# gisbi-kim/lt-mapper

Measured on AMD Instinct MI355X. Metric: keyframe-pairs/sec (removert+diff), higher is better.
Workload: dtype f32; 1 GPU; lot-2x500-os1-64-3res; sensor=os1-64

## Files before the change

### include/ltm.h

```cpp
#ifndef LTM_H
#define LTM_H

#include <stddef.h>
#include <stdint.h>

#ifdef __cplusplus
extern "C" {
#endif

#define LTM_ABI_VERSION 1

enum {
    LTM_OK = 0,
    LTM_E_INVALID = -1,
    LTM_E_DEVICE = -2,
    LTM_E_NOMEM = -3,
    LTM_E_UNSUPPORTED = -4
};

typedef struct ltm_ctx ltm_ctx;
typedef uint64_t ltm_cloud;
typedef uint64_t ltm_scanset;
typedef uint64_t ltm_poses;

// ... 158 lines not shown
int  ltm_icp_align_plane_scanset(ltm_ctx*, size_t n_pairs, ltm_search* const* targets, ltm_scanset sources, const uint32_t* source_kf ,
                                 const double* init16_or_null, const ltm_icp_params*, ltm_icp_result* results_host, double* trace_host_or_null);

int ltm_pose6d_to_affine3f(const float* xyzrpy , size_t n, float* affine12 );
int ltm_submaps_assemble(ltm_ctx*, ltm_scanset scans, const float* affine12_host_or_null ,
                         const int32_t* keys_host, size_t n_windows, int search_num, float leaf, int order, ltm_scanset* out);
int ltm_search_build_scanset(ltm_ctx*, ltm_scanset, size_t kf_begin, size_t kf_end, ltm_search** out );

typedef struct ltm_event ltm_event;
int  ltm_lane_create(ltm_ctx* parent, ltm_ctx** lane);
int  ltm_lane_fence(ltm_ctx* done_in, ltm_ctx* before_next_of);
int  ltm_event_record(ltm_ctx*, ltm_event** ev);
int  ltm_event_wait(ltm_ctx*, ltm_event* ev);
void ltm_event_destroy(ltm_event* ev);
int  ltm_cloud_lend(ltm_ctx* from, ltm_cloud h, ltm_ctx* to, ltm_cloud* out);
int  ltm_cloud_give(ltm_ctx* from, ltm_cloud h, ltm_ctx* to, ltm_cloud* out);
int  ltm_scanset_lend(ltm_ctx* from, ltm_scanset h, ltm_ctx* to, ltm_scanset* out);
int  ltm_scanset_give(ltm_ctx* from, ltm_scanset h, ltm_ctx* to, ltm_scanset* out);
int ltm_debug_range_image(ltm_ctx*, ltm_cloud pts, const double* T1, const double* T2, float res_alpha,
                          float* rimg, int32_t* ptidx);
int ltm_debug_viz_images(ltm_ctx*, ltm_cloud map, ltm_scanset scans, ltm_poses poses, size_t kf, float res_alpha, int mode,
                         float range_min, float range_max, float diff_min, float diff_max,
                         uint8_t* scan_bgr, uint8_t* map_bgr, uint8_t* diff_bgr, uint8_t* ptidx_bgr);
int ltm_debug_project(ltm_ctx*, const float* xyz, size_t n, float res_alpha, float* out_az_el_r, int32_t* out_row_col);
void ltm_rimg_size(float vfov, float hfov, float res_alpha, int* rows, int* cols);
int ltm_debug_selfcheck(ltm_ctx*, uint64_t* mismatches3, int* fast_math_enabled);
int ltm_debug_elevation_fit(float vfov_deg, float* c4, double* max_err_rad);
int ltm_debug_pcl_sort_order(const uint32_t* leaf_idx, size_t n, uint32_t* order_out, int use_std_sort, uint32_t* heap_sort_fallbacks );
int ltm_debug_voxel_key_bits(const float* mn3, const float* mx3, float leaf, uint64_t* kept_mask, unsigned* depth, double* frame_min3);
int ltm_debug_proj_launch(float vfov, float hfov, float res_alpha, const double* base2lidar16_or_null, size_t map_points, size_t n_keyframes, int on_device,
                          float* out_f32, uint32_t* out_u32, uint32_t first_block, size_t n_blocks, uint32_t* out_tile, uint32_t* out_kf);
int ltm_debug_vote_run_launch(size_t map_points, size_t n_keyframes, int tile_run, uint32_t first_block, size_t n_blocks, uint32_t* out_run, uint32_t* out_kf,
                              uint32_t* out_run_len, uint32_t* out_grid);
int ltm_debug_cull_check(ltm_ctx*, const float* xyz, size_t n, const double* inv_pose16_or_null, float res_alpha, uint64_t* violations);
int ltm_debug_cull_validation(ltm_ctx*, uint64_t* shapes_checked, uint64_t* shapes_failed);
int ltm_debug_occlusion_stats(ltm_ctx*, uint64_t* pairs, uint64_t* first_shell, uint64_t* projected, int reset);
int ltm_debug_voxel_stats(ltm_ctx*, uint64_t* grids, uint64_t* identity_hits, int reset);
int ltm_debug_knn_stats(ltm_ctx*, uint64_t* queries, uint64_t* undecided, uint64_t* two_phase_calls, uint64_t* unsorted_queue_calls, int reset);
int ltm_debug_sc_paths(int num_ring, int num_sector, int* scatter_in_lds, int* pair_in_lds);
int ltm_debug_cull_stats(ltm_ctx*, uint64_t* survivors, uint64_t* points, int reset);
int ltm_debug_pool_live(ltm_ctx*, uint64_t* live_blocks, uint64_t* live_bytes);

int ltm_profile_enable(ltm_ctx*, int on);
int ltm_profile_reset(ltm_ctx*);
int ltm_profile_read(ltm_ctx*, const char** names, double* ms, uint64_t* launches, double* units, double* bytes, int cap);
int ltm_profile_read_compulsory(ltm_ctx*, double* bytes_c, int cap);

#ifdef __cplusplus
}
#endif
#endif
```

### lt-mapper_amd/capi.py

```python
import ctypes as C
import os

import numpy as np

_HERE = os.path.dirname(os.path.abspath(__file__))
LIB_PATH = os.path.join(_HERE, "libltm_hip.so")

_lib = None

LTM_OK = 0
ERR_NAMES = {0: "LTM_OK", -1: "LTM_E_INVALID", -2: "LTM_E_DEVICE", -3: "LTM_E_NOMEM", -4: "LTM_E_UNSUPPORTED"}


class LtmError(RuntimeError):
    def __init__(self, code, msg):
        super().__init__(f"{ERR_NAMES.get(code, code)}: {msg}")
        self.code = code


class LtmConfig(C.Structure):
    _fields_ = [("vfov", C.c_float), ("hfov", C.c_float), ("lidar2base", C.c_double * 16),
                ("device", C.c_int), ("max_kf_batch", C.c_int)]


# ... 103 lines not shown
    "ltm_search_result_info": (_i, [_vp, _vp, _psz, _psz, C.POINTER(_vp), C.POINTER(_vp), C.POINTER(_vp)]),
    "ltm_search_result_free": (_i, [_vp, _vp]),
    "ltm_search_estimate_normals": (_i, [_vp, _sz, C.POINTER(_vp), _i, _vp]),
    "ltm_search_normals_info": (_i, [_vp, _vp, C.POINTER(_i), C.POINTER(_vp)]),
    "ltm_search_normals_download": (_i, [_vp, _vp, _vp]),
    "ltm_sc_default_params": (None, [C.POINTER(ScParams)]),
    "ltm_sc_from_scanset": (_i, [_vp, _u64, _sz, _sz, C.POINTER(ScParams), C.POINTER(_vp)]),
    "ltm_sc_from_descriptors": (_i, [_vp, _vp, _sz, C.POINTER(ScParams), C.POINTER(_vp)]),
    "ltm_sc_info": (_i, [_vp, _vp, _psz, C.POINTER(_i), C.POINTER(_i)]),
    "ltm_sc_download": (_i, [_vp, _vp, _vp, _vp, _vp]),
    "ltm_sc_distance": (_i, [_vp, _vp, _vp, _vp, _sz, C.POINTER(ScParams), _vp, _vp]),
    "ltm_sc_detect": (_i, [_vp, _vp, _vp, C.POINTER(ScParams), _vp, _vp, _vp, _vp, _vp]),
    "ltm_sc_free": (_i, [_vp, _vp]),
    "ltm_icp_default_params": (None, [C.POINTER(IcpParams)]),
    "ltm_icp_align": (_i, [_vp, _sz, C.POINTER(_vp), _pu64, _vp, C.POINTER(IcpParams), _vp, _vp]),
    "ltm_icp_align_scanset": (_i, [_vp, _sz, C.POINTER(_vp), _u64, _vp, _vp, C.POINTER(IcpParams), _vp, _vp]),
    "ltm_icp_align_plane": (_i, [_vp, _sz, C.POINTER(_vp), _pu64, _vp, C.POINTER(IcpParams), _vp, _vp]),
    "ltm_icp_align_plane_scanset": (_i, [_vp, _sz, C.POINTER(_vp), _u64, _vp, _vp, C.POINTER(IcpParams), _vp, _vp]),
    "ltm_pose6d_to_affine3f": (_i, [_vp, _sz, _vp]),
    "ltm_submaps_assemble": (_i, [_vp, _u64, _vp, _vp, _sz, _i, _f, _i, _pu64]),
    "ltm_search_build_scanset": (_i, [_vp, _u64, _sz, _sz, C.POINTER(_vp)]),
    "ltm_debug_pool_live": (_i, [_vp, _pu64, _pu64]),
    "ltm_debug_range_image": (_i, [_vp, _u64, _vp, _vp, _f, _vp, _vp]),
    "ltm_debug_viz_images": (_i, [_vp, _u64, _u64, _u64, _sz, _f, _i, _f, _f, _f, _f, _vp, _vp, _vp, _vp]),
    "ltm_debug_project": (_i, [_vp, _vp, _sz, _f, _vp, _vp]),
    "ltm_debug_elevation_fit": (_i, [_f, C.POINTER(_f), C.POINTER(C.c_double)]),
    "ltm_debug_pcl_sort_order": (_i, [C.POINTER(C.c_uint32), C.c_size_t, C.POINTER(C.c_uint32), _i, C.POINTER(C.c_uint32)]),
    "ltm_debug_voxel_key_bits": (_i, [C.POINTER(_f), C.POINTER(_f), _f, _pu64, C.POINTER(C.c_uint), C.POINTER(C.c_double)]),
    "ltm_debug_selfcheck": (_i, [_vp, _pu64, C.POINTER(_i)]),
    "ltm_debug_cull_check": (_i, [_vp, _vp, _sz, _vp, _f, _pu64]),
    "ltm_debug_cull_stats": (_i, [_vp, _pu64, _pu64, _i]),
    "ltm_debug_proj_launch": (_i, [_f, _f, _f, _vp, _sz, _sz, _i, _vp, _vp, C.c_uint32, _sz, _vp, _vp]),
    "ltm_debug_vote_run_launch": (_i, [_sz, _sz, _i, C.c_uint32, _sz, _vp, _vp, _vp, _vp]),
    "ltm_debug_cull_validation": (_i, [_vp, _pu64, _pu64]),
    "ltm_debug_occlusion_stats": (_i, [_vp, _pu64, _pu64, _pu64, _i]),
    "ltm_debug_voxel_stats": (_i, [_vp, _pu64, _pu64, _i]),
    "ltm_debug_knn_stats": (_i, [_vp, _pu64, _pu64, _pu64, _pu64, _i]),
    "ltm_debug_sc_paths": (_i, [_i, _i, C.POINTER(_i), C.POINTER(_i)]),
    "ltm_rimg_size": (None, [_f, _f, _f, C.POINTER(_i), C.POINTER(_i)]),
    "ltm_profile_enable": (_i, [_vp, _i]),
    "ltm_profile_reset": (_i, [_vp]),
    "ltm_profile_read_compulsory": (_i, [_vp, C.POINTER(C.c_double), _i]),
    "ltm_profile_read": (_i, [_vp, C.POINTER(C.c_char_p), C.POINTER(C.c_double), _pu64, C.POINTER(C.c_double),
                              C.POINTER(C.c_double), _i]),
}


def load_library(path=None):
    global _lib
    if _lib is not None and path is None:
        return _lib
    p = path or LIB_PATH
    try:
        import torch
    except Exception:
        pass
    if not os.path.exists(p):
        raise FileNotFoundError(
            f"{p} not found: build it with `make hip` (or __graft_entry__.build()). There is no CPU fallback.")
    lib = C.CDLL(p)
    for name, (res, args) in SIGNATURES.items():
        fn = getattr(lib, name)
        fn.restype = res
        fn.argtypes = args
    if path is None:
        _lib = lib
# ... 7 lines not shown
    if n < 0:
        raise ValueError("unsupported box / leaf")
    return n, mask.value, depth.value, np.array(list(fmin))


PROJ_LAUNCH_F32 = ("half_v", "half_h", "inv_v", "inv_h", "frows", "fcols", "row_max", "col_max", "row_scale", "col_scale", "row_bias", "col_bias",
                   "certain_lim", "rmin2", "eps", "el_tclamp")
PROJ_LAUNCH_U32 = ("rows", "cols", "npx", "steep_clamps", "packable", "n_tiles", "n_tg", "tg_magic", "tg_shift", "grid", "el_fit", "fast")


def proj_launch(vfov, hfov, alpha, base2lidar=None, map_points=0, n_keyframes=1, on_device=False, first_block=0, n_blocks=0):
    f = np.zeros(len(PROJ_LAUNCH_F32), dtype=np.float32)
    u = np.zeros(len(PROJ_LAUNCH_U32), dtype=np.uint32)
    tile = np.zeros(max(n_blocks, 1), dtype=np.uint32)
    kf = np.zeros(max(n_blocks, 1), dtype=np.uint32)
    b2l = None if base2lidar is None else _mat16(base2lidar)
    rc = load_library().ltm_debug_proj_launch(float(vfov), float(hfov), float(alpha), None if b2l is None else b2l.ctypes.data, int(map_points),
                                              int(n_keyframes), int(bool(on_device)), f.ctypes.data, u.ctypes.data, int(first_block), int(n_blocks),
                                              tile.ctypes.data, kf.ctypes.data)
    if rc != 0:
        raise LtmError(rc, "ltm_debug_proj_launch")
    return dict(zip(PROJ_LAUNCH_F32, f)), {k: int(v) for k, v in zip(PROJ_LAUNCH_U32, u)}, tile[:n_blocks], kf[:n_blocks]


def vote_run_launch(map_points, n_keyframes, tile_run, first_block=0, n_blocks=0):
    run = np.zeros(max(n_blocks, 1), dtype=np.uint32)
    kf = np.zeros(max(n_blocks, 1), dtype=np.uint32)
    run_len, grid = C.c_uint32(0), C.c_uint32(0)
    rc = load_library().ltm_debug_vote_run_launch(int(map_points), int(n_keyframes), int(tile_run), int(first_block), int(n_blocks), run.ctypes.data,
                                                  kf.ctypes.data, C.byref(run_len), C.byref(grid))
    if rc != 0:
        raise LtmError(rc, "ltm_debug_vote_run_launch")
    return run[:n_blocks], kf[:n_blocks], run_len.value, grid.value


def inverse4x4(m):
    a = np.ascontiguousarray(m, dtype=np.float64).reshape(16)
    out = np.empty(16, dtype=np.float64)
    if load_library().ltm_inverse4x4(a.ctypes.data, out.ctypes.data) != 0:
        raise ValueError("singular or non-finite matrix")
    return out.reshape(4, 4)


def pose6d_to_affine3f(xyzrpy):
    a = np.ascontiguousarray(xyzrpy, dtype=np.float32).reshape(-1, 6)
    out = np.empty((a.shape[0], 3, 4), dtype=np.float32)
    if a.shape[0] and load_library().ltm_pose6d_to_affine3f(a.ctypes.data, a.shape[0], out.ctypes.data) != 0:
        raise ValueError("ltm_pose6d_to_affine3f failed")
    return out


ORDERS = {"input": 0, "pcl": 1}


def _np_pts(a):
    a = np.ascontiguousarray(a, dtype=np.float32)
    if a.ndim != 2 or a.shape[1] != 4:
        a = a.reshape(-1, 4)
    return a


def _mat16(m):
    m = np.ascontiguousarray(m, dtype=np.float64).reshape(-1)
    assert m.size == 16
    return m

# ... 818 lines not shown
```

### lt-mapper_amd/csrc/ltm_api_vote.cpp

```cpp
#include "ltm_internal.h"

namespace ltm_detail {

static Geom geom_from(float vfov, float hfov, float alpha, int fast_math, int el_fit, const float* el_c, float cull_eps_scale, float cull_eps_floor)
{
    Geom g;
    g.vfov = vfov; g.hfov = hfov;
    g.rows = (int)roundf(vfov * alpha);
    g.cols = (int)roundf(hfov * alpha);
    g.fast = fast_math;
    const float ppd = std::max((float)g.rows / g.vfov, (float)g.cols / g.hfov);
    const float scale = cull_eps_scale > 0.0f ? cull_eps_scale : (el_fit ? 3.0e-4f : 6.0e-4f);
    g.cull_eps_px = std::max(cull_eps_floor, scale * ppd);
    g.el_fit = el_fit;
    for (int i = 0; i < 4; ++i) g.el_c[i] = el_c[i];
    const double out_deg = std::min(2.0, (double)g.vfov / std::max(g.rows, 1));
    g.el_tclamp = (float)std::tan((0.5 * (double)g.vfov + out_deg) * (3.14159265358979323846 / 180.0));
    return g;
}
Geom geom_for(const ltm_ctx* c, float alpha)
{
    return geom_from(c->cfg.vfov, c->cfg.hfov, alpha, c->fast_math, c->el_fit, c->el_c, c->cull_eps_scale, c->cull_eps_floor);
}

// ... 528 lines not shown
    return guarded(c, [&] { if (shapes_checked) *shapes_checked = c->cull_geoms_checked; if (shapes_failed) *shapes_failed = c->cull_geoms_failed; });
}

int ltm_debug_proj_launch(float vfov, float hfov, float alpha, const double* base2lidar16, size_t map_points, size_t n_keyframes, int on_device,
                          float* out_f32, uint32_t* out_u32, uint32_t first_block, size_t n_blocks, uint32_t* out_tile, uint32_t* out_kf)
{
    if (!(vfov > 0.0f) || !(hfov > 0.0f) || !(alpha > 0.0f) || !out_f32 || !out_u32 || (n_blocks && (!out_tile || !out_kf))) return LTM_E_INVALID;
    if (map_points >= 0xffffffffull || n_keyframes >= 0xffffffffull) return LTM_E_INVALID;
    float el_c[4];
    double err = 0.0;
    const int el_fit = elevation_fit_for(vfov, el_c, &err);
    const Geom g = geom_from(vfov, hfov, alpha, 0, el_fit, el_c, 0.0f, 1.0e-3f);
    if (g.rows <= 0 || g.cols <= 0) return LTM_E_INVALID;
    HostMat34 b2l{};
    b2l.m[0] = b2l.m[5] = b2l.m[10] = 1.0;
    int ident = 1;
    if (base2lidar16) { b2l = to34(base2lidar16); ident = mat_is_identity(base2lidar16) ? 1 : 0; }
    if (proj_launch_debug(g, b2l, ident, map_points, n_keyframes, on_device, out_f32, out_u32) != hipSuccess) return LTM_E_DEVICE;
    if (n_blocks) proj_launch_blocks(map_points, n_keyframes, first_block, n_blocks, out_tile, out_kf);
    return LTM_OK;
}

int ltm_debug_vote_run_launch(size_t map_points, size_t n_keyframes, int tile_run, uint32_t first_block, size_t n_blocks, uint32_t* out_run, uint32_t* out_kf,
                              uint32_t* out_run_len, uint32_t* out_grid)
{
    if (map_points >= 0xffffffffull || n_keyframes >= 0xffffffffull || tile_run < 1 || (n_blocks && (!out_run || !out_kf))) return LTM_E_INVALID;
    uint32_t len = 0;
    const unsigned grid = vote_run_launch_blocks(map_points, n_keyframes, tile_run, first_block, n_blocks, out_run, out_kf, &len);
    if (out_run_len) *out_run_len = len;
    if (out_grid) *out_grid = grid;
    return LTM_OK;
}

int ltm_debug_cull_stats(ltm_ctx* c, uint64_t* survivors, uint64_t* points, int reset)
{
    return guarded(c, [&] {
        unsigned long long v[2] = {0, 0};
        LTM_HIP(cull_stats(v, reset, c->stream, c->kopts.stats_blockmin));
        if (survivors) *survivors = v[0];
        if (points) *points = v[1];
    });
}

int ltm_debug_occlusion_stats(ltm_ctx* c, uint64_t* pairs, uint64_t* first_shell, uint64_t* projected, int reset)
{
    return guarded(c, [&] {
        if (pairs) *pairs = c->occl_pairs;
        if (first_shell) *first_shell = c->occl_near;
        if (projected) *projected = c->occl_far_live;
        if (reset) { c->occl_pairs = 0; c->occl_near = 0; c->occl_far_live = 0; }
    });
}

}
```

### lt-mapper_amd/csrc/ltm_k_projection.hip

```cpp
#include "ltm_kernels_common.h"
#include <rocprim/device/device_scan.hpp>
#include <rocprim/iterator/transform_iterator.hpp>

namespace ltm {

__global__ void k_fill_u32(uint32_t* p, uint32_t v, size_t n)
{
    size_t i = (size_t)blockIdx.x * blockDim.x + threadIdx.x;
    const size_t stride = (size_t)gridDim.x * blockDim.x;
    for (; i < n; i += stride) p[i] = v;
}
__global__ void k_fill_u64(uint64_t* p, uint64_t v, size_t n)
{
    size_t i = (size_t)blockIdx.x * blockDim.x + threadIdx.x;
    const size_t stride = (size_t)gridDim.x * blockDim.x;
    for (; i < n; i += stride) p[i] = v;
}
hipError_t fill_u32(uint32_t* p, uint32_t v, size_t n, hipStream_t s)
{
    if (!n) return hipSuccess;
    k_fill_u32<<<dim3((unsigned)std::min<size_t>(grid_for(n), 8192)), dim3(kBlock), 0, s>>>(p, v, n);
    return hipGetLastError();
}
hipError_t fill_u64(uint64_t* p, uint64_t v, size_t n, hipStream_t s)
// ... 394 lines not shown
    bool alive = false;
    if (tile < n_tiles) alive = !tile_out_of_reach(approx_poses + 16 * (size_t)(kb + kfb), tile_bounds + 6 * (size_t)tile, u2f(smax_bits[kfb]), thr);
    __shared__ uint32_t wsum[kBlock / 64];
    const uint64_t b = __builtin_amdgcn_ballot_w64(alive);
    if ((threadIdx.x & 63u) == 0u) wsum[threadIdx.x >> 6] = (uint32_t)__popcll(b);
    __syncthreads();
    if (threadIdx.x == 0) {
        uint32_t t = 0;
        for (int w = 0; w < kBlock / 64; ++w) t += wsum[w];
        if (t) atomicAdd(live, (unsigned long long)t);
    }
}
hipError_t count_live_tiles(const float* approx_poses_dev, size_t kb, size_t nb, const float* tile_bounds_dev, size_t n_tiles,
                            const uint32_t* smax_bits_dev, float thr, unsigned long long* live_dev, hipStream_t s)
{
    if (!nb || !n_tiles) return hipSuccess;
    k_count_live_tiles<<<dim3(grid_for(n_tiles), (unsigned)nb), dim3(kBlock), 0, s>>>(approx_poses_dev, (uint32_t)kb, (uint32_t)nb, tile_bounds_dev,
                                                                                    (uint32_t)n_tiles, smax_bits_dev, thr, live_dev);
    return hipGetLastError();
}

static constexpr int kCullSlots = 512;

template <bool B2L_IDENTITY, bool EL3>
__global__ void __launch_bounds__(kBlock) __attribute__((amdgpu_waves_per_eu(8, 8)))
k_vote_map_cull(const float4* __restrict__ map, uint32_t M, const double* __restrict__ inv_poses, const float* __restrict__ approx_poses,
                uint32_t kb, uint32_t nb, HostMat34 b2l_h, ProjLaunch pl, RunLaunch rl, const float* __restrict__ qbound_img,
                const float* __restrict__ tile_bounds, const uint32_t* __restrict__ smax_bits, float thr, uint64_t* __restrict__ img)
{
    __shared__ uint64_t vals[kCullSlots];
    __shared__ uint32_t tags[kCullSlots];
    __shared__ uint32_t queue[kCullQueue];
    __shared__ uint16_t uqueue[kCullQueue];
    __shared__ uint32_t qcount, ucount;
    static_assert(kMaxTileRun * kBlock * kPtsPerThread <= 65536, "uqueue entries are 16 bits");
    const uint32_t per_block = (uint32_t)(kBlock * kPtsPerThread);
    const RunKf rk = run_kf_of_block(blockIdx.x, rl, nb);
    if (!rk.valid) return;
    const RimgGeom& g = pl.g;
    const uint32_t npx = pl.npx;
    const uint32_t kf = kb + rk.kfb;
    const uint32_t first_tile = rk.run * rl.T;
    const uint32_t run_base = first_tile * per_block;
    uint64_t* __restrict__ imgk = img + (size_t)rk.kfb * npx;
    const float* __restrict__ qk = qbound_img + (size_t)rk.kfb * npx;
    const float* __restrict__ ap = approx_poses + 16 * (size_t)kf;
    uint32_t todo;
    {
        const uint32_t t = threadIdx.x & 63u;
        bool visit = (t < rl.T) & (first_tile + t < pl.n_tiles);
        if (visit && tile_bounds) visit = !tile_out_of_reach(ap, tile_bounds + 6 * (size_t)(first_tile + t), u2f(smax_bits[rk.kfb]), thr);
        todo = (uint32_t)__builtin_amdgcn_ballot_w64(visit);
    }
    if (!todo) return;
    for (int s = threadIdx.x; s < kCullSlots; s += kBlock) { tags[s] = kEmptyTag; vals[s] = ~0ull; }
    if (threadIdx.x == 0) { qcount = 0; ucount = 0; }
    __syncthreads();
    const bool fast_ok = pl.packable & ((f2u(ap[15]) << 1) != 0u);
    const double* __restrict__ inv_pose = inv_poses + 12 * (size_t)kf;
    bool flush = false;
    uint32_t qbase = 0;
    for (; todo; todo &= todo - 1u) {
        const uint32_t tile = first_tile + (uint32_t)__builtin_ctz(todo);
        const uint32_t block_base = tile * per_block;
        const float4* __restrict__ mapb = map + block_base;
        const uint32_t nloc = min(per_block, M - block_base);
        const bool full_tile = (nloc == per_block) & fast_ok;
        if (full_tile) {
            constexpr int kInFlight = 4;
            constexpr bool kPrefetch = true;
            float4 nxt[kInFlight];
            if (kPrefetch) {
#pragma unroll
                for (int u = 0; u < kInFlight; ++u) nxt[u] = mapb[(uint32_t)u * kBlock + threadIdx.x];
            }
            const uint32_t lane_word = threadIdx.x << 20;
#pragma unroll
            for (uint32_t j0 = 0; j0 < (uint32_t)kPtsPerThread; j0 += kInFlight) {
                float4 pt[kInFlight];
                CullCand cc[kInFlight];
                float q0[kInFlight];
#pragma unroll
                for (int u = 0; u < kInFlight; ++u) {
                    const uint32_t li = (j0 + u) * kBlock + threadIdx.x;
                    if (kPrefetch) {
                        pt[u] = nxt[u];
                        if (j0 + kInFlight < (uint32_t)kPtsPerThread) nxt[u] = mapb[li + kInFlight * kBlock];
                    } else {
                        pt[u] = mapb[li];
                    }
                }
#pragma unroll
                for (int u = 0; u < kInFlight; ++u) {
                    bool ok;
                    const float3 p = xform_approx(ap, pt[u], ok);
                    cc[u] = cull_candidates<EL3>(pl, p);
                    cc[u].unusual |= cc[u].multi | (B2L_IDENTITY ? false : (cc[u].r2 < pl.rmin2));
                    q0[u] = *reinterpret_cast<const float*>(reinterpret_cast<const char*>(qk) + ((__umul24((uint32_t)cc[u].rb, (uint32_t)g.cols) + (uint32_t)cc[u].cb) << 2));
                }
                bool mt[kInFlight];
#pragma unroll
                for (int u = 0; u < kInFlight; ++u) {
                    mt[u] = cc[u].unusual | (cc[u].r2 < q0[u]);
                }
                const uint64_t b0 = __builtin_amdgcn_ballot_w64(mt[0]), b1 = __builtin_amdgcn_ballot_w64(mt[1]),
                               b2 = __builtin_amdgcn_ballot_w64(mt[2]), b3 = __builtin_amdgcn_ballot_w64(mt[3]);
                const uint32_t n0 = (uint32_t)__popcll(b0), n1 = (uint32_t)__popcll(b1), n2 = (uint32_t)__popcll(b2), n3 = (uint32_t)__popcll(b3);
                const uint32_t total = n0 + n1 + n2 + n3;
                if (total) {
                    uint32_t base = 0;
                    if ((threadIdx.x & 63u) == 0u) base = atomicAdd(&qcount, total);
                    base = (uint32_t)__builtin_amdgcn_readfirstlane((int)base) - qbase;
                    if (base + total <= (uint32_t)kCullQueue) {
                        const uint64_t bal[kInFlight] = {b0, b1, b2, b3};
                        const uint32_t off[kInFlight] = {0u, n0, n0 + n1, n0 + n1 + n2};
#pragma unroll
                        for (int u = 0; u < kInFlight; ++u) {
                            if (!mt[u]) continue;
                            const uint32_t below = __builtin_amdgcn_mbcnt_hi((uint32_t)(bal[u] >> 32), __builtin_amdgcn_mbcnt_lo((uint32_t)bal[u], 0u));
                            const uint32_t rowq = cc[u].unusual ? 511u : (uint32_t)cc[u].rb;
                            queue[base + off[u] + below] = (((rowq << 11) | (uint32_t)cc[u].cb) | lane_word) | (((j0 + u) * kBlock) << 20);
                        }
                    }
                }
            }
        }
        const uint32_t nu_waiting = (uint32_t)__builtin_amdgcn_readfirstlane((int)ucount);
        __syncthreads();
        const uint32_t qend = (uint32_t)__builtin_amdgcn_readfirstlane((int)qcount);
        const uint32_t nq_all = full_tile ? qend - qbase : (uint32_t)kCullQueue + 1u;
        qbase = qend;
        if (nloc == per_block && threadIdx.x == 0 && (blockIdx.x & 63u) == 0u) {
            atomicAdd(&g_cull_stats[0], (unsigned long long)nq_all);
            atomicAdd(&g_cull_stats[1], (unsigned long long)nloc);
        }
        if (nq_all) {
            flush = true;
            const Mat34 Tinv = load_mat(inv_pose);
            if (__builtin_expect(nq_all > (uint32_t)kCullQueue, 0)) {
                for (uint32_t li = threadIdx.x; li < nloc; li += kBlock)
                    exact_insert<B2L_IDENTITY, 8, 64>(map, block_base + li, Tinv, b2l_h, g, vals, tags, imgk);
            } else {
                if (__builtin_expect(nu_waiting + nq_all > (uint32_t)kCullQueue, 0)) {
                    uint32_t q0 = threadIdx.x;
                    asm volatile("" : "+v"(q0));
                    for (uint32_t q = q0; q < nu_waiting; q += kBlock)
                        exact_insert<B2L_IDENTITY, 8, 64>(map, run_base + uqueue[q], Tinv, b2l_h, g, vals, tags, imgk);
                    __syncthreads();
                    if (threadIdx.x == 0) ucount = 0;
                    __syncthreads();
                }
                const uint32_t tile_word = (tile - first_tile) << 12;
                for (uint32_t q = threadIdx.x; q < nq_all; q += kBlock) {
                    const uint32_t e = queue[q];
                    const int row = (int)((e >> 11) & 511u), col = (int)(e & 2047u);
                    if (row == 511) { uqueue[atomicAdd(&ucount, 1u)] = (uint16_t)(tile_word | (e >> 20)); continue; }
                    const uint32_t i = block_base + (e >> 20);
                    const uint32_t px = (uint32_t)(row * g.cols + col);
                    const uint64_t v = ((uint64_t)exact_range_bits<B2L_IDENTITY>(map[i], Tinv, b2l_h) << 32) | (uint64_t)i;
                    const int slot = table_claim<8, 64>(tags, row, col, px);
                    if (slot >= 0) { if (v < vals[slot]) atomicMin(reinterpret_cast<unsigned long long*>(&vals[slot]), (unsigned long long)v); }
                    else img_min_u64(imgk + px, v);
                }
            }
        }
        __builtin_amdgcn_s_waitcnt(0x0f70);
        __syncthreads();
    }
    if (!flush) return;
    const uint32_t nu = ucount;
    if (nu) {
        const Mat34 Tinv = load_mat(inv_pose);
        for (uint32_t q = threadIdx.x; q < nu; q += kBlock)
            exact_insert<B2L_IDENTITY, 8, 64>(map, run_base + uqueue[q], Tinv, b2l_h, g, vals, tags, imgk);
    }
    __syncthreads();
    for (int s = threadIdx.x; s < kCullSlots; s += kBlock) {
        const uint32_t t = tags[s];
        if (t != kEmptyTag) img_min_u64(imgk + t, vals[s]);
    }
}

hipError_t cull_stats(unsigned long long* out2, int reset, hipStream_t s, int which_kernel)
{
    hipError_t e = hipMemcpyFromSymbolAsync(out2, HIP_SYMBOL(g_cull_stats), 16, 16 * (size_t)(which_kernel ? 1 : 0), hipMemcpyDeviceToHost, s);
    if (e != hipSuccess) return e;
    e = hipStreamSynchronize(s);
    if (e != hipSuccess || !reset) return e;
    const unsigned long long z[4] = {0, 0, 0, 0};
    e = hipMemcpyToSymbolAsync(HIP_SYMBOL(g_cull_stats), z, 32, 0, hipMemcpyHostToDevice, s);
    return e == hipSuccess ? hipStreamSynchronize(s) : e;
}


hipError_t vote_map_range_images(const float4* map, size_t M, const double* inv_poses_dev, const float* approx_poses_dev, size_t kb, size_t nb,
                                 HostMat34 b2l, int b2l_identity, Geom g, const float* qbound_img, const float* tile_bounds_dev,
                                 const uint32_t* smax_bits_dev, float thr, int mode, uint64_t* map_img, hipStream_t s, const KernelOpts& ko)
{
    if (!M || !nb) return hipSuccess;
    if (mode != 0 || !ko.vote_cull || !approx_poses_dev || !qbound_img) return map_range_images(map, M, inv_poses_dev, approx_poses_dev, kb, nb, b2l, b2l_identity, g, map_img, s, ko);
    const ProjLaunch pl = make_proj_launch(g, b2l, b2l_identity, M);
    const RunLaunch rl = make_run_launch(pl.n_tiles, (uint32_t)std::max(ko.vote_tile_run, 1));
    dim3 grid(run_kf_grid(rl, nb));
// ... 553 lines not shown
        if (e != hipSuccess) return e;
    }
    proj_launch_flatten(pl, (uint32_t)nb, f, u);
    return hipSuccess;
}
void proj_launch_blocks(size_t M, size_t nb, uint32_t first_block, size_t n, uint32_t* tile, uint32_t* kf)
{
    Geom g{};
    g.vfov = g.hfov = 1.0f;
    const ProjLaunch pl = make_proj_launch(g, HostMat34{}, 1, M);
    for (size_t i = 0; i < n; ++i) {
        const TileKf t = tile_kf_of_block(first_block + (uint32_t)i, pl, (uint32_t)nb);
        tile[i] = t.valid ? t.tile : 0xffffffffu;
        kf[i] = t.valid ? t.kfb : 0xffffffffu;
    }
}
size_t vote_run_blocks(size_t M, size_t nb, int tile_run)
{
    const size_t per_block = (size_t)kBlock * kPtsPerThread;
    return (size_t)make_run_launch((uint32_t)((M + per_block - 1) / per_block), (uint32_t)std::max(tile_run, 1)).n_runs * nb;
}
unsigned vote_run_launch_blocks(size_t M, size_t nb, int tile_run, uint32_t first_block, size_t n, uint32_t* run, uint32_t* kf, uint32_t* run_len)
{
    const size_t per_block = (size_t)kBlock * kPtsPerThread;
    const RunLaunch rl = make_run_launch((uint32_t)((M + per_block - 1) / per_block), (uint32_t)std::max(tile_run, 1));
    for (size_t i = 0; i < n; ++i) {
        const RunKf t = run_kf_of_block(first_block + (uint32_t)i, rl, (uint32_t)nb);
        run[i] = t.valid ? t.run : 0xffffffffu;
        kf[i] = t.valid ? t.kfb : 0xffffffffu;
    }
    if (run_len) *run_len = rl.T;
    return run_kf_grid(rl, nb);
}

}
```

### lt-mapper_amd/csrc/ltm_kernels.h

```cpp
#pragma once
#include <hip/hip_runtime_api.h>
#include <stddef.h>
#include <stdint.h>

namespace ltm {

struct Geom {
    float vfov, hfov;
    int rows, cols;
    int fast;
    float cull_eps_px;
    int el_fit;
    float el_c[4];
    float el_tclamp;
};

struct HostMat34 { double m[12]; };

static const uint32_t kNoPointBits = 0x461C4000u;

hipError_t fill_u32(uint32_t* p, uint32_t v, size_t n, hipStream_t s);
hipError_t fill_u64(uint64_t* p, uint64_t v, size_t n, hipStream_t s);

hipError_t scan_range_images(const float4* scans, const uint64_t* offsets_dev, size_t kb, size_t nb,
// ... 2 lines not shown
hipError_t scan_range_images_multi(const float4* scans, const uint64_t* offsets_dev, size_t kb, size_t nb, uint64_t n_pts, uint64_t max_kf_pts, Geom g,
                                   int n_shapes, const int* rows, const int* cols, uint32_t* const* imgs, uint32_t* const* smax_bits, hipStream_t s);
hipError_t scan_qbound(const uint32_t* scan_img, size_t n, float thr, float* qbound, hipStream_t s);
hipError_t tile_bounds(const float4* map, size_t M, float* bounds, hipStream_t s);
hipError_t subtile_bounds(const float4* map, size_t M, float* bounds, hipStream_t s);
struct KernelOpts {
    int map_kernel_variant = 2;
    int vote_cull = 1;
    int tile_cull = 1;
    int vote_tile_run = 4;
    int stats_blockmin = 0;
};
hipError_t map_range_images(const float4* map, size_t M, const double* inv_poses_dev, const float* approx_poses_dev, size_t kb, size_t nb,
                            HostMat34 b2l, int b2l_identity, Geom g, uint64_t* map_img, hipStream_t s, const KernelOpts& ko);
hipError_t occlusion_shell_pairs(const float* approx_poses_dev, size_t kb, size_t nb, const float* tile_bounds_dev, size_t n_tiles, Geom g, float r_lo, float r_hi,
                                 const uint64_t* img, int use_cmax, uint32_t* cmax, uint8_t* done, uint8_t* flags, uint32_t* pos, uint32_t* list, uint32_t* count,
                                 void* temp, size_t temp_bytes, hipStream_t s, uint32_t* dirty_rows = nullptr,
                                 const float* sub_bounds_dev = nullptr, uint8_t* submask = nullptr, unsigned long long* sub_stats = nullptr);
hipError_t map_range_images_pairs(const float4* map, size_t M, const double* inv_poses_dev, const float* approx_poses_dev, size_t kb, size_t nb,
                                  HostMat34 b2l, int b2l_identity, Geom g, uint64_t* map_img, const uint32_t* pairs, size_t n_pairs, hipStream_t s, const KernelOpts& ko,
                                  const uint8_t* submask = nullptr);
hipError_t compare_and_flag(const uint32_t* scan_img, const uint64_t* map_img, size_t n_px_total, float thr, int mode,
                            uint8_t* labels, hipStream_t s);
hipError_t vote_map_range_images(const float4* map, size_t M, const double* inv_poses_dev, const float* approx_poses_dev, size_t kb, size_t nb,
                                 HostMat34 b2l, int b2l_identity, Geom g, const float* qbound_img, const float* tile_bounds_dev,
                                 const uint32_t* smax_bits_dev, float thr, int mode, uint64_t* map_img, hipStream_t s, const KernelOpts& ko);
hipError_t count_live_tiles(const float* approx_poses_dev, size_t kb, size_t nb, const float* tile_bounds_dev, size_t n_tiles,
                            const uint32_t* smax_bits_dev, float thr, unsigned long long* live_dev, hipStream_t s);
static constexpr int kProjLaunchFloats = 16, kProjLaunchWords = 12;
hipError_t proj_launch_debug(Geom g, HostMat34 b2l, int b2l_identity, size_t M, size_t nb, int on_device, float* f, uint32_t* u);
void proj_launch_blocks(size_t M, size_t nb, uint32_t first_block, size_t n, uint32_t* tile, uint32_t* kf);
size_t vote_run_blocks(size_t M, size_t nb, int tile_run);
unsigned vote_run_launch_blocks(size_t M, size_t nb, int tile_run, uint32_t first_block, size_t n, uint32_t* run, uint32_t* kf, uint32_t* run_len);
hipError_t cull_stats(unsigned long long* out2, int reset, hipStream_t s, int which_kernel);
hipError_t cull_check(const float* xyz_dev, size_t n, const HostMat34* T, const HostMat34* b2l, int b2l_identity, const float* approx_pose_dev,
                      Geom g, unsigned long long* bad_dev, hipStream_t s);
hipError_t cull_probe_points(Geom g, size_t n, const HostMat34* pose, float* xyz_dev, hipStream_t s);
hipError_t single_range_image(const float4* pts, size_t n, const HostMat34* T1, const HostMat34* T2, Geom g,
                              uint64_t* img, hipStream_t s);
hipError_t decode_image(const uint64_t* img, size_t npx, float* rimg, int32_t* ptidx, hipStream_t s);
hipError_t viz_diff(const uint32_t* scan_bits, const float* map_r, size_t n, int mode, float* out, hipStream_t s);
hipError_t viz_colormap_f32(const float* src, size_t n, float a, float b, const uint8_t* lut, uint8_t* bgr, hipStream_t s);
hipError_t viz_colormap_i32(const int32_t* src, size_t n, double a, double b, const uint8_t* lut, uint8_t* bgr, hipStream_t s);
hipError_t debug_project(const float* xyz_dev, size_t n, Geom g, float* az_el_r, int32_t* row_col, hipStream_t s);
hipError_t selfcheck_fast_math(float vfov, float hfov, unsigned long long* counts_dev, hipStream_t s);

size_t scan_temp_bytes(size_t n);
hipError_t exclusive_scan_u8(const uint8_t* labels, uint32_t* pos, size_t n, void* temp, size_t temp_bytes, hipStream_t s);
hipError_t exclusive_scan_img_valid(const uint64_t* img, uint32_t* pos, size_t n, void* temp, size_t temp_bytes, hipStream_t s);
hipError_t exclusive_scan_u32(const uint32_t* in, uint32_t* out, size_t n, void* temp, size_t temp_bytes, hipStream_t s);
hipError_t partition_scatter(const float4* in, const uint8_t* labels, const uint32_t* pos, size_t n,
                             float4* kept, float4* flagged, hipStream_t s);
hipError_t reproject_gather(const uint64_t* img, const uint32_t* pos, size_t npx, size_t nb, const float4* map,
                            const double* inv_poses_dev, size_t kb, HostMat34 b2l, int b2l_identity,
                            float4* out, hipStream_t s);
hipError_t image_bounds(const uint32_t* pos, const uint64_t* img, size_t npx, size_t nb, uint32_t* out, hipStream_t s);
hipError_t flag_bounds(const uint32_t* pos, const uint8_t* flag, size_t n, const uint64_t* offsets_dev, size_t kf0, uint64_t first, size_t nb,
                       uint32_t* out, hipStream_t s);
hipError_t gather_u32(const uint32_t* in, const uint64_t* idx_dev, size_t m, size_t n, uint32_t tail_value_index_n,
                      uint32_t* out, hipStream_t s);

hipError_t transform_cloud(const float4* in, size_t n, const HostMat34* t1, const HostMat34* t2, float4* out, hipStream_t s);
hipError_t transform_scans(const float4* in, const uint64_t* offsets_dev, size_t n_kf, uint64_t n_pts,
                           HostMat34 first, int first_identity, const double* per_kf_dev, float4* out, hipStream_t s);
hipError_t zip_concat(const float4* a, const uint64_t* oa, const float4* b, const uint64_t* ob, const float4* c, const uint64_t* oc,
                      const uint64_t* out_off_dev, size_t n_kf, uint64_t n, float4* out, hipStream_t s);
// ... 143 lines not shown
```

### lt-mapper_amd/csrc/ltm_kernels_common.h

```cpp
#pragma once
#include "ltm_kernels.h"
#include "ltm_device_math.h"
#include "ltm_device_prims.h"

#include <algorithm>
#include <cstring>
#include <type_traits>
#include <hip/hip_runtime.h>

namespace ltm {

static constexpr int kBlock = 256;

__host__ __device__ inline RimgGeom make_geom(Geom g)
{
    RimgGeom r;
    r.vfov = g.vfov; r.hfov = g.hfov;
    r.half_v = g.vfov / 2.0f; r.half_h = g.hfov / 2.0f;
    r.inv_v = 1.0f / g.vfov; r.inv_h = 1.0f / g.hfov;
    r.fast = g.fast != 0;
    r.eps = g.cull_eps_px;
    r.el_c0 = g.el_c[0]; r.el_c1 = g.el_c[1]; r.el_c2 = g.el_c[2]; r.el_c3 = g.el_c[3]; r.el_tclamp = g.el_tclamp; r.el_fit = g.el_fit != 0;
    r.rows = g.rows; r.cols = g.cols;
    r.frows = (float)g.rows; r.fcols = (float)g.cols;
    r.row_max = (float)(g.rows - 1); r.col_max = (float)(g.cols - 1);
    return r;
}

static constexpr unsigned kKfPerTile = 8;
struct ProjLaunch {
    RimgGeom g;
    float row_scale, col_scale;
    float row_bias, col_bias;
    float certain_lim;
    float rmin2;
    uint32_t npx;
    uint32_t n_tiles, n_tg;
    uint32_t tg_magic, tg_shift;
    bool steep_clamps;
    bool packable;
};
__host__ __device__ inline void group_quotient_magic(uint32_t n_groups, uint32_t& magic, uint32_t& shift)
{
    const uint32_t d = n_groups ? n_groups : 1u;
    uint32_t s = 0;
    while (((uint64_t)1 << s) < d) ++s;
    shift = s;
    magic = (uint32_t)((((uint64_t)1 << (26u + s)) / d) + 1u);
}
__host__ __device__ inline ProjLaunch make_proj_launch(Geom gg, const HostMat34& b2l, int b2l_identity, size_t M)
{
    ProjLaunch pl;
    const RimgGeom g = make_geom(gg);
    pl.g = g;
    pl.row_scale = g.frows * (57.29577951308232f / g.vfov); pl.col_scale = g.fcols * (57.29577951308232f / g.hfov);
    pl.row_bias = 0.5f * g.frows + 0.5f - g.eps; pl.col_bias = 0.5f * g.fcols + 0.5f - g.eps;
    pl.certain_lim = 1.0f - 2.0f * g.eps;
    float rmin = 0.0f;
    if (!b2l_identity) {
        const float tx = (float)b2l.m[3], ty = (float)b2l.m[7], tz = (float)b2l.m[11];
        rmin = 0.125f * __builtin_sqrtf(tx * tx + ty * ty + tz * tz) + 1.0e-6f;
    }
    pl.rmin2 = rmin * rmin;
    pl.npx = (uint32_t)(g.rows * g.cols);
    pl.steep_clamps = g.vfov < 88.0f;
    pl.packable = g.rows < 511 && g.cols <= 2048;
    const size_t per_block = (size_t)kBlock * 16;
    pl.n_tiles = (uint32_t)((M + per_block - 1) / per_block);
    pl.n_tg = (pl.n_tiles + 7u) >> 3;
    group_quotient_magic(pl.n_tg, pl.tg_magic, pl.tg_shift);
    return pl;
}

struct TileKf { uint32_t tile, kfb; bool valid; };
__host__ __device__ inline TileKf tile_kf_of_block(uint32_t b, const ProjLaunch& pl, uint32_t nb)
{
    static_assert(kKfPerTile == 8, "the shifts below are log2(8 XCDs) + log2(kKfPerTile)");
    const uint32_t x = b & 7u, kfl = (b >> 3) & (kKfPerTile - 1u), q = b >> 6;
    const uint32_t kg = (uint32_t)(((uint64_t)(b & ~63u) * pl.tg_magic) >> 32) >> pl.tg_shift;
    const uint32_t tg = q - kg * pl.n_tg;
    TileKf t;
    t.tile = tg * 8u + x;
    t.kfb = kg * kKfPerTile + kfl;
    t.valid = (t.tile < pl.n_tiles) & (t.kfb < nb);
    return t;
}
static inline unsigned tile_kf_grid(size_t n_tiles, size_t nb)
{
    const size_t n_tg = (n_tiles + 7) / 8, n_kg = (nb + kKfPerTile - 1) / kKfPerTile;
    return (unsigned)(n_tg * 8 * kKfPerTile * n_kg);
}

static constexpr uint32_t kMaxTileRun = 16;
struct RunLaunch {
    uint32_t T;
    uint32_t n_runs, n_rg;
    uint32_t rg_magic, rg_shift;
};
__host__ __device__ inline RunLaunch make_run_launch(uint32_t n_tiles, uint32_t T)
// ... 66 lines not shown
```

Baseline: 3296 keyframe-pairs/s.

## Use per-wave vote queues with deferred drain instead of per-tile block syncs

The cull/vote kernel no longer processes each tile followed by block-wide __syncthreads and a shared queue counter. Each wave now keeps its own queue segment in shared memory, storing a packed pixel index plus tile/group/lane bits. The segment is drained only when nearly full or at the end, and loads for the next group are prefetched across tile boundaries. This removes block barriers and the shared atomic counter per tile, and partial tiles fall back to exact insertion. In exchange it adds magic-division row/col decoding and a new queueability limit on pixel count, plus a debug API to check the word encoding.

```diff
diff --git a/include/ltm.h b/include/ltm.h
--- a/include/ltm.h
+++ b/include/ltm.h
@@ -214,6 +214,7 @@
                           float* out_f32, uint32_t* out_u32, uint32_t first_block, size_t n_blocks, uint32_t* out_tile, uint32_t* out_kf);
 int ltm_debug_vote_run_launch(size_t map_points, size_t n_keyframes, int tile_run, uint32_t first_block, size_t n_blocks, uint32_t* out_run, uint32_t* out_kf,
                               uint32_t* out_run_len, uint32_t* out_grid);
+int ltm_debug_vote_queue_word(float vfov, float hfov, float res_alpha, uint32_t* out_u32, size_t n_px, const uint32_t* px, uint32_t* out_row, uint32_t* out_col);
 int ltm_debug_cull_check(ltm_ctx*, const float* xyz, size_t n, const double* inv_pose16_or_null, float res_alpha, uint64_t* violations);
 int ltm_debug_cull_validation(ltm_ctx*, uint64_t* shapes_checked, uint64_t* shapes_failed);
 int ltm_debug_occlusion_stats(ltm_ctx*, uint64_t* pairs, uint64_t* first_shell, uint64_t* projected, int reset);
diff --git a/lt-mapper_amd/capi.py b/lt-mapper_amd/capi.py
--- a/lt-mapper_amd/capi.py
+++ b/lt-mapper_amd/capi.py
@@ -159,6 +159,7 @@
     "ltm_debug_cull_stats": (_i, [_vp, _pu64, _pu64, _i]),
     "ltm_debug_proj_launch": (_i, [_f, _f, _f, _vp, _sz, _sz, _i, _vp, _vp, C.c_uint32, _sz, _vp, _vp]),
     "ltm_debug_vote_run_launch": (_i, [_sz, _sz, _i, C.c_uint32, _sz, _vp, _vp, _vp, _vp]),
+    "ltm_debug_vote_queue_word": (_i, [C.c_float, C.c_float, C.c_float, _vp, _sz, _vp, _vp, _vp]),
     "ltm_debug_cull_validation": (_i, [_vp, _pu64, _pu64]),
     "ltm_debug_occlusion_stats": (_i, [_vp, _pu64, _pu64, _pu64, _i]),
     "ltm_debug_voxel_stats": (_i, [_vp, _pu64, _pu64, _i]),
@@ -232,6 +233,21 @@
     if rc != 0:
         raise LtmError(rc, "ltm_debug_vote_run_launch")
     return run[:n_blocks], kf[:n_blocks], run_len.value, grid.value
+
+
+VOTE_QUEUE_WORD_U32 = ("rows", "cols", "npx", "fast_path", "px_magic", "px_shift", "px_bits", "npx_limit")
+
+
+def vote_queue_word(vfov, hfov, alpha, px=None):
+    u = np.zeros(len(VOTE_QUEUE_WORD_U32), dtype=np.uint32)
+    p = np.ascontiguousarray(np.zeros(0) if px is None else px, dtype=np.uint32)
+    row = np.zeros(max(len(p), 1), dtype=np.uint32)
+    col = np.zeros(max(len(p), 1), dtype=np.uint32)
+    rc = load_library().ltm_debug_vote_queue_word(float(vfov), float(hfov), float(alpha), u.ctypes.data, len(p), p.ctypes.data if len(p) else None,
+                                                  row.ctypes.data, col.ctypes.data)
+    if rc != 0:
+        raise LtmError(rc, "ltm_debug_vote_queue_word")
+    return {k: int(v) for k, v in zip(VOTE_QUEUE_WORD_U32, u)}, row[:len(p)], col[:len(p)]
 
 
 def inverse4x4(m):
diff --git a/lt-mapper_amd/csrc/ltm_api_vote.cpp b/lt-mapper_amd/csrc/ltm_api_vote.cpp
--- a/lt-mapper_amd/csrc/ltm_api_vote.cpp
+++ b/lt-mapper_amd/csrc/ltm_api_vote.cpp
@@ -584,6 +584,20 @@
     return LTM_OK;
 }
 
+int ltm_debug_vote_queue_word(float vfov, float hfov, float alpha, uint32_t* out_u32, size_t n_px, const uint32_t* px, uint32_t* out_row, uint32_t* out_col)
+{
+    if (!(vfov > 0.0f) || !(hfov > 0.0f) || !(alpha > 0.0f) || !out_u32 || (n_px && (!px || !out_row || !out_col))) return LTM_E_INVALID;
+    float el_c[4];
+    double err = 0.0;
+    const int el_fit = elevation_fit_for(vfov, el_c, &err);
+    const Geom g = geom_from(vfov, hfov, alpha, 0, el_fit, el_c, 0.0f, 1.0e-3f);
+    if (g.rows <= 0 || g.cols <= 0) return LTM_E_INVALID;
+    for (size_t i = 0; i < n_px; ++i)
+        if (px[i] >= (1u << 26)) return LTM_E_INVALID;
+    vote_queue_word_debug(g, out_u32, n_px, px, out_row, out_col);
+    return LTM_OK;
+}
+
 int ltm_debug_cull_stats(ltm_ctx* c, uint64_t* survivors, uint64_t* points, int reset)
 {
     return guarded(c, [&] {
diff --git a/lt-mapper_amd/csrc/ltm_k_projection.hip b/lt-mapper_amd/csrc/ltm_k_projection.hip
--- a/lt-mapper_amd/csrc/ltm_k_projection.hip
+++ b/lt-mapper_amd/csrc/ltm_k_projection.hip
@@ -450,8 +450,12 @@
     __shared__ uint32_t tags[kCullSlots];
     __shared__ uint32_t queue[kCullQueue];
     __shared__ uint16_t uqueue[kCullQueue];
-    __shared__ uint32_t qcount, ucount;
+    __shared__ uint32_t ucount;
     static_assert(kMaxTileRun * kBlock * kPtsPerThread <= 65536, "uqueue entries are 16 bits");
+    static_assert(kMaxTileRun <= 16 && kPtsPerThread == 16 && kBlock == 256, "queue word: 4 bits of tile, 4 of group, 6 of lane; the wave is implied");
+    constexpr int kInFlight = 4;
+    constexpr uint32_t kSeg = (uint32_t)kCullQueue / (kBlock / 64);
+    constexpr uint32_t kDrainAt = kSeg - 64u * kInFlight;
     const uint32_t per_block = (uint32_t)(kBlock * kPtsPerThread);
     const RunKf rk = run_kf_of_block(blockIdx.x, rl, nb);
     if (!rk.valid) return;
@@ -472,121 +476,122 @@
     }
     if (!todo) return;
     for (int s = threadIdx.x; s < kCullSlots; s += kBlock) { tags[s] = kEmptyTag; vals[s] = ~0ull; }
-    if (threadIdx.x == 0) { qcount = 0; ucount = 0; }
+    if (threadIdx.x == 0) ucount = 0;
     __syncthreads();
-    const bool fast_ok = pl.packable & ((f2u(ap[15]) << 1) != 0u);
+    uint32_t full = todo;
+    {
+        const uint32_t t_last = pl.n_tiles - 1u - first_tile;
+        if (t_last < kMaxTileRun && (M & (per_block - 1u)) != 0u) full &= ~(1u << t_last);
+    }
+    const uint32_t fast = (pl.vote_queueable & ((f2u(ap[15]) << 1) != 0u)) ? full : 0u;
+    const uint32_t slow = todo & ~fast;
+    const bool sampled = (blockIdx.x & 63u) == 0u;
+    if (sampled && threadIdx.x == 0) atomicAdd(&g_cull_stats[1], (unsigned long long)((uint32_t)__popc(full) * per_block));
     const double* __restrict__ inv_pose = inv_poses + 12 * (size_t)kf;
-    bool flush = false;
-    uint32_t qbase = 0;
-    for (; todo; todo &= todo - 1u) {
-        const uint32_t tile = first_tile + (uint32_t)__builtin_ctz(todo);
-        const uint32_t block_base = tile * per_block;
-        const float4* __restrict__ mapb = map + block_base;
-        const uint32_t nloc = min(per_block, M - block_base);
-        const bool full_tile = (nloc == per_block) & fast_ok;
-        if (full_tile) {
-            constexpr int kInFlight = 4;
-            constexpr bool kPrefetch = true;
-            float4 nxt[kInFlight];
-            if (kPrefetch) {
-#pragma unroll
-                for (int u = 0; u < kInFlight; ++u) nxt[u] = mapb[(uint32_t)u * kBlock + threadIdx.x];
+    const float4* __restrict__ mapr = map + run_base;
+    uint32_t* __restrict__ seg = queue + (uint32_t)__builtin_amdgcn_readfirstlane((int)(threadIdx.x >> 6)) * kSeg;
+    const uint32_t lane = threadIdx.x & 63u;
+    const uint32_t wave_off = threadIdx.x & 192u;
+    bool more = fast != 0u;
+    uint32_t G = 0, rest = 0, nq = 0, nsurv = 0;
+    float4 nxt[kInFlight];
+    if (more) {
+        G = (uint32_t)__builtin_ctz(fast) << 2;
+        rest = fast & (fast - 1u);
+#pragma unroll
+        for (int u = 0; u < kInFlight; ++u) nxt[u] = mapr[(G << 10) + (uint32_t)u * kBlock + threadIdx.x];
+    }
+    for (;;) {
+        if (__builtin_expect((nq > kDrainAt) | !more, 0)) {
+            __builtin_amdgcn_fence(__ATOMIC_ACQ_REL, "wavefront");
+            const Mat34 Tinv = load_mat(inv_pose);
+            for (uint32_t q = lane; q < nq; q += 64u) {
+                const uint32_t e = seg[q];
+                const uint32_t off = ((e >> 24) << 8) | wave_off | ((e >> kVoteQueuePxBits) & 63u);
+                const uint32_t px = e & kVoteQueuePxUncertain;
+                if (px == kVoteQueuePxUncertain) {
+                    const uint32_t ticket = atomicAdd(&ucount, 1u);
+                    if (ticket < (uint32_t)kCullQueue) uqueue[ticket] = (uint16_t)off;
+                    else exact_insert<B2L_IDENTITY, 8, 64>(map, run_base + off, Tinv, b2l_h, g, vals, tags, imgk);
+                    continue;
+                }
+                const uint32_t i = run_base + off;
+                uint32_t row, col;
+                vote_queue_row_col(px, (uint32_t)g.cols, pl.px_magic, pl.px_shift, row, col);
+                const uint64_t v = ((uint64_t)exact_range_bits<B2L_IDENTITY>(map[i], Tinv, b2l_h) << 32) | (uint64_t)i;
+                const int slot = table_claim<8, 64>(tags, (int)row, (int)col, px);
+                if (slot >= 0) { if (v < vals[slot]) atomicMin(reinterpret_cast<unsigned long long*>(&vals[slot]), (unsigned long long)v); }
+                else img_min_u64(imgk + px, v);
             }
-            const uint32_t lane_word = threadIdx.x << 20;
-#pragma unroll
-            for (uint32_t j0 = 0; j0 < (uint32_t)kPtsPerThread; j0 += kInFlight) {
-                float4 pt[kInFlight];
-                CullCand cc[kInFlight];
-                float q0[kInFlight];
-#pragma unroll
-                for (int u = 0; u < kInFlight; ++u) {
-                    const uint32_t li = (j0 + u) * kBlock + threadIdx.x;
-                    if (kPrefetch) {
-                        pt[u] = nxt[u];
-                        if (j0 + kInFlight < (uint32_t)kPtsPerThread) nxt[u] = mapb[li + kInFlight * kBlock];
-                    } else {
-                        pt[u] = mapb[li];
-                    }
-                }
-#pragma unroll
-                for (int u = 0; u < kInFlight; ++u) {
-                    bool ok;
-                    const float3 p = xform_approx(ap, pt[u], ok);
-                    cc[u] = cull_candidates<EL3>(pl, p);
-                    cc[u].unusual |= cc[u].multi | (B2L_IDENTITY ? false : (cc[u].r2 < pl.rmin2));
-                    q0[u] = *reinterpret_cast<const float*>(reinterpret_cast<const char*>(qk) + ((__umul24((uint32_t)cc[u].rb, (uint32_t)g.cols) + (uint32_t)cc[u].cb) << 2));
-                }
-                bool mt[kInFlight];
-#pragma unroll
-                for (int u = 0; u < kInFlight; ++u) {
-                    mt[u] = cc[u].unusual | (cc[u].r2 < q0[u]);
-                }
-                const uint64_t b0 = __builtin_amdgcn_ballot_w64(mt[0]), b1 = __builtin_amdgcn_ballot_w64(mt[1]),
-                               b2 = __builtin_amdgcn_ballot_w64(mt[2]), b3 = __builtin_amdgcn_ballot_w64(mt[3]);
-                const uint32_t n0 = (uint32_t)__popcll(b0), n1 = (uint32_t)__popcll(b1), n2 = (uint32_t)__popcll(b2), n3 = (uint32_t)__popcll(b3);
-                const uint32_t total = n0 + n1 + n2 + n3;
-                if (total) {
-                    uint32_t base = 0;
-                    if ((threadIdx.x & 63u) == 0u) base = atomicAdd(&qcount, total);
-                    base = (uint32_t)__builtin_amdgcn_readfirstlane((int)base) - qbase;
-                    if (base + total <= (uint32_t)kCullQueue) {
-                        const uint64_t bal[kInFlight] = {b0, b1, b2, b3};
-                        const uint32_t off[kInFlight] = {0u, n0, n0 + n1, n0 + n1 + n2};
-#pragma unroll
-                        for (int u = 0; u < kInFlight; ++u) {
-                            if (!mt[u]) continue;
-                            const uint32_t below = __builtin_amdgcn_mbcnt_hi((uint32_t)(bal[u] >> 32), __builtin_amdgcn_mbcnt_lo((uint32_t)bal[u], 0u));
-                            const uint32_t rowq = cc[u].unusual ? 511u : (uint32_t)cc[u].rb;
-                            queue[base + off[u] + below] = (((rowq << 11) | (uint32_t)cc[u].cb) | lane_word) | (((j0 + u) * kBlock) << 20);
-                        }
-                    }
-                }
+            nsurv += nq;
+            nq = 0;
+            __builtin_amdgcn_s_waitcnt(0x0f70);
+            if (more) {
+#pragma unroll
+                for (int u = 0; u < kInFlight; ++u) nxt[u] = mapr[(G << 10) + (uint32_t)u * kBlock + threadIdx.x];
             }
         }
-        const uint32_t nu_waiting = (uint32_t)__builtin_amdgcn_readfirstlane((int)ucount);
-        __syncthreads();
-        const uint32_t qend = (uint32_t)__builtin_amdgcn_readfirstlane((int)qcount);
-        const uint32_t nq_all = full_tile ? qend - qbase : (uint32_t)kCullQueue + 1u;
-        qbase = qend;
-        if (nloc == per_block && threadIdx.x == 0 && (blockIdx.x & 63u) == 0u) {
-            atomicAdd(&g_cull_stats[0], (unsigned long long)nq_all);
-            atomicAdd(&g_cull_stats[1], (unsigned long long)nloc);
-        }
-        if (nq_all) {
-            flush = true;
-            const Mat34 Tinv = load_mat(inv_pose);
-            if (__builtin_expect(nq_all > (uint32_t)kCullQueue, 0)) {
-                for (uint32_t li = threadIdx.x; li < nloc; li += kBlock)
-                    exact_insert<B2L_IDENTITY, 8, 64>(map, block_base + li, Tinv, b2l_h, g, vals, tags, imgk);
-            } else {
-                if (__builtin_expect(nu_waiting + nq_all > (uint32_t)kCullQueue, 0)) {
-                    uint32_t q0 = threadIdx.x;
-                    asm volatile("" : "+v"(q0));
-                    for (uint32_t q = q0; q < nu_waiting; q += kBlock)
-                        exact_insert<B2L_IDENTITY, 8, 64>(map, run_base + uqueue[q], Tinv, b2l_h, g, vals, tags, imgk);
-                    __syncthreads();
-                    if (threadIdx.x == 0) ucount = 0;
-                    __syncthreads();
-                }
-                const uint32_t tile_word = (tile - first_tile) << 12;
-                for (uint32_t q = threadIdx.x; q < nq_all; q += kBlock) {
-                    const uint32_t e = queue[q];
-                    const int row = (int)((e >> 11) & 511u), col = (int)(e & 2047u);
-                    if (row == 511) { uqueue[atomicAdd(&ucount, 1u)] = (uint16_t)(tile_word | (e >> 20)); continue; }
-                    const uint32_t i = block_base + (e >> 20);
-                    const uint32_t px = (uint32_t)(row * g.cols + col);
-                    const uint64_t v = ((uint64_t)exact_range_bits<B2L_IDENTITY>(map[i], Tinv, b2l_h) << 32) | (uint64_t)i;
-                    const int slot = table_claim<8, 64>(tags, row, col, px);
-                    if (slot >= 0) { if (v < vals[slot]) atomicMin(reinterpret_cast<unsigned long long*>(&vals[slot]), (unsigned long long)v); }
-                    else img_min_u64(imgk + px, v);
-                }
+        if (!more) break;
+        float4 pt[kInFlight];
+        CullCand cc[kInFlight];
+        float q0[kInFlight];
+        uint32_t pxi[kInFlight];
+#pragma unroll
+        for (int u = 0; u < kInFlight; ++u) pt[u] = nxt[u];
+        float3 p[kInFlight];
+#pragma unroll
+        for (int u = 0; u < kInFlight; ++u) {
+            bool ok;
+            p[u] = xform_approx(ap, pt[u], ok);
+        }
+        const uint32_t Gcur = G;
+        if ((G & 3u) != 3u) ++G;
+        else if (rest) { G = (uint32_t)__builtin_ctz(rest) << 2; rest &= rest - 1u; }
+        else more = false;
+#pragma unroll
+        for (int u = 0; u < kInFlight; ++u) nxt[u] = mapr[(G << 10) + (uint32_t)u * kBlock + threadIdx.x];
+#pragma unroll
+        for (int u = 0; u < kInFlight; ++u) {
+            cc[u] = cull_candidates<EL3>(pl, p[u]);
+            cc[u].unusual |= cc[u].multi | (B2L_IDENTITY ? false : (cc[u].r2 < pl.rmin2));
+            pxi[u] = __umul24((uint32_t)cc[u].rb, (uint32_t)g.cols) + (uint32_t)cc[u].cb;
+            q0[u] = *reinterpret_cast<const float*>(reinterpret_cast<const char*>(qk) + (pxi[u] << 2));
+        }
+        bool mt[kInFlight];
+#pragma unroll
+        for (int u = 0; u < kInFlight; ++u) {
+            mt[u] = cc[u].unusual | (cc[u].r2 < q0[u]);
+        }
+        const uint64_t b0 = __builtin_amdgcn_ballot_w64(mt[0]), b1 = __builtin_amdgcn_ballot_w64(mt[1]),
+                       b2 = __builtin_amdgcn_ballot_w64(mt[2]), b3 = __builtin_amdgcn_ballot_w64(mt[3]);
+        const uint32_t n0 = (uint32_t)__popcll(b0), n1 = (uint32_t)__popcll(b1), n2 = (uint32_t)__popcll(b2), n3 = (uint32_t)__popcll(b3);
+        const uint32_t total = n0 + n1 + n2 + n3;
+        if (total) {
+            const uint64_t bal[kInFlight] = {b0, b1, b2, b3};
+            const uint32_t off[kInFlight] = {nq, nq + n0, nq + n0 + n1, nq + n0 + n1 + n2};
+            const uint32_t word = (Gcur << 26) | (lane << kVoteQueuePxBits);
+#pragma unroll
+            for (int u = 0; u < kInFlight; ++u) {
+                if (!mt[u]) continue;
+                const uint32_t below = __builtin_amdgcn_mbcnt_hi((uint32_t)(bal[u] >> 32), __builtin_amdgcn_mbcnt_lo((uint32_t)bal[u], 0u));
+                seg[off[u] + below] = (word | ((uint32_t)u << 24)) | (cc[u].unusual ? kVoteQueuePxUncertain : pxi[u]);
             }
-        }
-        __builtin_amdgcn_s_waitcnt(0x0f70);
-        __syncthreads();
-    }
-    if (!flush) return;
-    const uint32_t nu = ucount;
+            nq += total;
+        }
+    }
+    if (__builtin_expect(slow != 0u, 0)) {
+        const Mat34 Tinv = load_mat(inv_pose);
+        for (uint32_t sl = slow; sl; sl &= sl - 1u) {
+            const uint32_t block_base = (first_tile + (uint32_t)__builtin_ctz(sl)) * per_block;
+            const uint32_t nloc = min(per_block, M - block_base);
+            for (uint32_t li = threadIdx.x; li < nloc; li += kBlock)
+                exact_insert<B2L_IDENTITY, 8, 64>(map, block_base + li, Tinv, b2l_h, g, vals, tags, imgk);
+            if (nloc == per_block) nsurv += per_block / (kBlock / 64);
+        }
+    }
+    if (sampled && lane == 0u && nsurv) atomicAdd(&g_cull_stats[0], (unsigned long long)nsurv);
+    __syncthreads();
+    const uint32_t nu = min(ucount, (uint32_t)kCullQueue);
     if (nu) {
         const Mat34 Tinv = load_mat(inv_pose);
         for (uint32_t q = threadIdx.x; q < nu; q += kBlock)
@@ -1206,5 +1211,13 @@
     if (run_len) *run_len = rl.T;
     return run_kf_grid(rl, nb);
 }
-
-}
+void vote_queue_word_debug(Geom g, uint32_t* u, size_t n, const uint32_t* px, uint32_t* row, uint32_t* col)
+{
+    HostMat34 b2l{};
+    const ProjLaunch pl = make_proj_launch(g, b2l, 1, 0);
+    const uint32_t uu[kVoteQueueWords] = {(uint32_t)pl.g.rows, (uint32_t)pl.g.cols, pl.npx, pl.vote_queueable ? 1u : 0u, pl.px_magic, pl.px_shift, kVoteQueuePxBits, kVoteQueuePxLimit};
+    memcpy(u, uu, sizeof uu);
+    for (size_t i = 0; i < n; ++i) vote_queue_row_col(px[i], (uint32_t)pl.g.cols, pl.px_magic, pl.px_shift, row[i], col[i]);
+}
+
+}
diff --git a/lt-mapper_amd/csrc/ltm_kernels.h b/lt-mapper_amd/csrc/ltm_kernels.h
--- a/lt-mapper_amd/csrc/ltm_kernels.h
+++ b/lt-mapper_amd/csrc/ltm_kernels.h
@@ -58,6 +58,8 @@
 void proj_launch_blocks(size_t M, size_t nb, uint32_t first_block, size_t n, uint32_t* tile, uint32_t* kf);
 size_t vote_run_blocks(size_t M, size_t nb, int tile_run);
 unsigned vote_run_launch_blocks(size_t M, size_t nb, int tile_run, uint32_t first_block, size_t n, uint32_t* run, uint32_t* kf, uint32_t* run_len);
+static constexpr int kVoteQueueWords = 8;
+void vote_queue_word_debug(Geom g, uint32_t* u, size_t n, const uint32_t* px, uint32_t* row, uint32_t* col);
 hipError_t cull_stats(unsigned long long* out2, int reset, hipStream_t s, int which_kernel);
 hipError_t cull_check(const float* xyz_dev, size_t n, const HostMat34* T, const HostMat34* b2l, int b2l_identity, const float* approx_pose_dev,
                       Geom g, unsigned long long* bad_dev, hipStream_t s);
diff --git a/lt-mapper_amd/csrc/ltm_kernels_common.h b/lt-mapper_amd/csrc/ltm_kernels_common.h
--- a/lt-mapper_amd/csrc/ltm_kernels_common.h
+++ b/lt-mapper_amd/csrc/ltm_kernels_common.h
@@ -39,7 +39,17 @@
     uint32_t tg_magic, tg_shift;
     bool steep_clamps;
     bool packable;
+    bool vote_queueable;
+    uint32_t px_magic, px_shift;
 };
+static constexpr uint32_t kVoteQueuePxBits = 18u;
+static constexpr uint32_t kVoteQueuePxUncertain = (1u << kVoteQueuePxBits) - 1u;
+static constexpr uint32_t kVoteQueuePxLimit = kVoteQueuePxUncertain;
+__host__ __device__ inline void vote_queue_row_col(uint32_t px, uint32_t cols, uint32_t px_magic, uint32_t px_shift, uint32_t& row, uint32_t& col)
+{
+    row = (uint32_t)(((uint64_t)(px << 6) * px_magic) >> 32) >> px_shift;
+    col = px - row * cols;
+}
 __host__ __device__ inline void group_quotient_magic(uint32_t n_groups, uint32_t& magic, uint32_t& shift)
 {
     const uint32_t d = n_groups ? n_groups : 1u;
@@ -65,6 +75,8 @@
     pl.npx = (uint32_t)(g.rows * g.cols);
     pl.steep_clamps = g.vfov < 88.0f;
     pl.packable = g.rows < 511 && g.cols <= 2048;
+    pl.vote_queueable = g.rows > 0 && g.cols > 0 && (uint64_t)g.rows * (uint64_t)g.cols <= kVoteQueuePxLimit;
+    group_quotient_magic((uint32_t)g.cols, pl.px_magic, pl.px_shift);
     const size_t per_block = (size_t)kBlock * 16;
     pl.n_tiles = (uint32_t)((M + per_block - 1) / per_block);
     pl.n_tg = (pl.n_tiles + 7u) >> 3;
```

Measured after the change: 3390 keyframe-pairs/s, median of 6. 2.8% higher.
